# ShuoYangRobotics/Cerberus

Measured on NVIDIA H100. Metric: sliding-window solves/sec (10-frame x 150-feature windows), higher is better.
Workload: dtype f64

## Files before the change

### cerberus_b200/csrc/solve_kernel.cuh

```cuda
#pragma once
#include "eval_kernels.cuh"

namespace cerb {

#if defined(CERB_PHASE_TIMING) && !defined(CERB_CUSIM)
__device__ unsigned long long g_phase_cycles[48];
#define PH_DECL() long long ph_t = clock64()
#define PH_MARK_T(id, t) do { if ((threadIdx.x & 31) == 0) { const long long ph_n = clock64(); if (threadIdx.x == (t)) atomicAdd(&g_phase_cycles[id], (unsigned long long)(ph_n - ph_t)); ph_t = ph_n; } __syncwarp(); } while (0)
#define PH_MARK(id) PH_MARK_T(id, 0)
#define PH_ARG , long long &ph_t
#define PH_FWD , ph_t
#else
#define PH_DECL()
#define PH_MARK_T(id, t)
#define PH_MARK(id)
#define PH_ARG
#define PH_FWD
#endif

enum { CERB_WINDOW = 10, NX = 79, NYB = 13, NFR = 11, NY = 143, NR = 222, NRP = 224, HXX_SZ = 79 * 79, HXY_SZ = 79 * 143, X_TD = 78, SOLVE_THREADS = 256, FT = 64, TILE_LD = 33, NOBS_PLANES = 9 };
enum { HBLK = NYB * NYB, AD_SZ = NFR * HBLK, BO_SZ = (NFR - 1) * HBLK };
#ifndef CERB_SOLVE_MIN_BLOCKS
#define CERB_SOLVE_MIN_BLOCKS 1
#endif
// ... 53 lines not shown
    double *red;
    double *wj;
    double *sca;
    double *chain_col;
    double *idg;
    double *idx;
    int *ti;
    unsigned long long *mbar;
    double *tile;
};
enum { S_RADIUS = 0, S_MU, S_REUSE, S_XCOST, S_CCOST, S_ALPHA, S_GNORM2, S_GNNORM2, S_GDOTGN, S_MODEL, S_STEPNORM, S_XNORM, S_DLNORM,
       S_OK, S_DONE, S_TERM, S_ITER, S_NSUCC, S_INVALID, S_GMAX, S_INIT_COST, S_P, S_Q, S_VHV, S_LCOST, S_LNORM, S_LGMAX, S_COUNT };
static_assert(S_COUNT <= 32, "scalar slots overlap the chain's column line");
enum { TI_PRIOR_MAP = 0, TI_NCHUNKS = 96, TI_CHUNK_CACHE = 97, TI_CACHED_CHUNKS = 15, TI_CHAIN_DONE = 130, TI_IMU_MASK = 131, TI_INTS = 132 };
static_assert(TI_PRIOR_MAP + CERB_MAX_PRIOR_DIM <= TI_NCHUNKS && TI_CHUNK_CACHE + 2 * TI_CACHED_CHUNKS <= TI_CHAIN_DONE && TI_IMU_MASK < TI_INTS && TI_INTS % 2 == 0,
              "s.ti slots overlap");
enum { SMEM_DOUBLES = HXX_SZ + SMEM_HXX_PAD + HXY_SZ + AD_SZ + BO_SZ + 7 * NRP + 2 * ST_STRIDE + 99 + 18 + 3 + 31 * 39 + 960 + 192 + 8 * 256 + 128 * 8 + 32 + 32 + TI_INTS / 2 + 144 + 80 };

CERB_D void smem_carve(double *base, Smem &s) {
    double *p = base;
    s.Hxx = p; p += HXX_SZ; s.mbar = reinterpret_cast<unsigned long long *>(p + 1); p += SMEM_HXX_PAD; s.Hxy = p; p += HXY_SZ; s.Ad = p; p += AD_SZ; s.Bo = p; p += BO_SZ;
    s.g = p; p += NRP; s.sc = p; p += NRP; s.D = p; p += NRP; s.gh = p; p += NRP; s.gn = p; p += NRP; s.stp = p; p += NRP; s.yv = p; p += NRP;
    s.xs = p; p += ST_STRIDE; s.xc = p; p += ST_STRIDE;
    s.Rw = p; p += 99; s.Rex = p; p += 18; p += 3;
    s.Ju = p; p += 31 * 39; s.red = p; p += 8 * 256; s.wj = p; p += 128 * 8;
    s.lin = p; p += 960; s.pdx = p; p += 96; s.pr = p; p += 96; s.sca = p; p += 32; s.chain_col = p; p += 32;
    s.ti = reinterpret_cast<int *>(p); p += TI_INTS / 2;
    s.idg = p; p += 144;
    s.idx = p; p += 80;
    s.tile = s.Hxy;
}

template <int NV>
CERB_D void block_sum(const double *v, double *red, double *out, int tid) {
    for (int k = 0; k < NV; k++) red[k * 256 + tid] = v[k];
    __syncthreads();
    for (int s = 128; s > 0; s >>= 1) {
        if (tid < s) for (int k = 0; k < NV; k++) red[k * 256 + tid] += red[k * 256 + tid + s];
        __syncthreads();
    }
    for (int k = 0; k < NV; k++) out[k] = red[k * 256];
    __syncthreads();
}

CERB_D void copy_g2s(double *dst, const double *src, int n, int tid) {
    for (int k0 = tid; k0 < n; k0 += 8 * SOLVE_THREADS) {
        double b[8];
        _Pragma("unroll")
        for (int u = 0; u < 8; u++) { const int k = k0 + u * SOLVE_THREADS; b[u] = (k < n) ? src[k] : 0.0; }
        _Pragma("unroll")
        for (int u = 0; u < 8; u++) { const int k = k0 + u * SOLVE_THREADS; if (k < n) dst[k] = b[u]; }
    }
}
CERB_D void copy_g2s_async(double *dst, const double *src, int n, int tid) {
    for (int k = tid; k < n; k += SOLVE_THREADS) CERB_CP_ASYNC8(dst + k, src + k);
}
CERB_D void load_geometry(const double *x, Smem &s, int tid) {
    if (tid < 11) { const m33 R = qtoR(ldq(x + ST_POSE + 7 * tid + 3)); for (int k = 0; k < 9; k++) s.Rw[9 * tid + k] = R.m[k]; }
    else if (tid < 13) { const int e = tid - 11; const m33 R = qtoR(ldq(x + ST_EX + 7 * e + 3)); for (int k = 0; k < 9; k++) s.Rex[9 * e + k] = R.m[k]; }
    __syncthreads();
}

struct ObsCtx { int start, nobs, off; double lam, pix, piy, vix, viy, tdi; };

struct ObsVals { double px, py, vx, vy, td; int stereo; };
CERB_D void obs_fetch(const double *obs, const int *stereo, int mo, int o, int cam, ObsVals &v) {
    v.px = obs[(cam ? 4 : 0) * mo + o]; v.py = obs[(cam ? 5 : 1) * mo + o]; v.vx = obs[(cam ? 6 : 2) * mo + o]; v.vy = obs[(cam ? 7 : 3) * mo + o];
    v.td = obs[8 * mo + o]; v.stereo = stereo[o];
}

CERB_NOINLINE double vision_cost(const SolveParams &P, int w, const double *x, const double *lam, int tid) {
    CERB_DYN_SMEM(double, smem_base);
    Smem s; smem_carve(smem_base, s);
    const int nF = P.n_features[w], mo = P.maxObs;
    const double *obs = P.obs + (size_t)w * NOBS_PLANES * P.maxObs;
    const int *stereo = P.obs_stereo + (size_t)w * P.maxObs;
    double cost = 0.0;
    for (int idx = tid; idx < 4 * nF; idx += SOLVE_THREADS) {
        const int f = idx >> 2, cam = idx & 1, part = (idx >> 1) & 1;
        ObsCtx c;
        c.start = P.feat_start[(size_t)w * P.maxF + f]; c.nobs = P.feat_nobs[(size_t)w * P.maxF + f]; c.off = P.feat_off[(size_t)w * P.maxF + f];
        c.lam = lam[f];
        c.pix = obs[0 * mo + c.off]; c.piy = obs[1 * mo + c.off]; c.vix = obs[2 * mo + c.off]; c.viy = obs[3 * mo + c.off];
        c.tdi = obs[8 * mo + c.off];
        const int k0 = part ? 6 : 0, k1 = part ? c.nobs : (c.nobs < 6 ? c.nobs : 6);
        const double inv_l = 1.0 / c.lam;
        const int i = c.start;
        const d3 tic = ld3(x + ST_EX);
        const double tdv = x[ST_TD];
        const d3 pts_i_td = mk3(c.pix, c.piy, 1.0) - (tdv - c.tdi) * mk3(c.vix, c.viy, 0.0);
        const d3 p_bi = mv33(ldm33(s.Rex), inv_l * pts_i_td) + tic;
        const d3 p_w = mv33(ldm33(s.Rw + 9 * i), p_bi) + ld3(x + ST_POSE + 7 * i);
        const double *Rcp = cam ? s.Rex + 9 : s.Rex;
        const d3 tc = cam ? ld3(x + ST_EX + 7) : tic;
        ObsVals cur, nxt;
        cur.px = cur.py = cur.vx = cur.vy = cur.td = 0.0; cur.stereo = 0;
        if (k0 < k1) obs_fetch(obs, stereo, mo, c.off + k0, cam, cur);
        _Pragma("unroll 1")
        for (int k = k0; k < k1; k++) {
            nxt = cur;
            if (k + 1 < k1) obs_fetch(obs, stereo, mo, c.off + k + 1, cam, nxt);
            const bool k3 = (k == 0);
            const bool on = k3 ? (cam == 1 && cur.stereo) : (cam == 0 || cur.stereo);
            if (on) {
                const int j = c.start + k;
                const d3 p_bj = k3 ? p_bi : mTv33(ldm33(s.Rw + 9 * j), p_w - ld3(x + ST_POSE + 7 * j));
                const d3 p_cj = mTv33(ldm33(Rcp), p_bj - tc);
                const double iz = 1.0 / p_cj.z;
                const double r0 = P.sqrt_info * (p_cj.x * iz - (cur.px - (tdv - cur.td) * cur.vx));
// ... 243 lines not shown
            PH_MARK(29);
            __syncthreads();
            PH_MARK(22);
            if (jbase >= 0) {
                _Pragma("unroll")
                for (int fj = 0; fj < 2; fj++) {
                    const int jf = j0 + fj;
                    if (jf >= NFR || jf == a) continue;
                    const double *q = jp + (4 * fj) * VJ_SZ + tid;
                    smem_base[jbase + jca * a + jcj * jf] += ((q[0] + q[VJ_SZ]) + q[2 * VJ_SZ]) + q[3 * VJ_SZ];
                }
            }
            PH_MARK(23);
        }
        __syncthreads();
        {
            double *ex = T;
            ex[0 * 256 + tid] = h; ex[1 * 256 + tid] = gq; ex[2 * 256 + tid] = wT;
            for (int k = 0; k < 6; k++) { ex[(3 + k) * 256 + tid] = wI[k]; ex[(9 + k) * 256 + tid] = wE0[k]; ex[(15 + k) * 256 + tid] = wE1[k]; }
        }
        __syncthreads();
        for (int e = tid; e < VP_SZ; e += SOLVE_THREADS) {
            double v = 0.0;
            for (int wq = 0; wq < 8; wq++) v += ((wq < 5) ? s.Ju + 8 * VJ_SZ + VP_SZ * wq : s.tile + VT_SZ + VP_SZ * (wq - 5))[e];
            const int blk = e >> 6, ra = (e >> 3) & 7, rb = e & 7;
            const int ga = blk < 3 ? 0 : (blk < 5 ? 2 : 3), gb = blk == 0 ? 0 : (blk == 1 || blk == 3 ? 2 : 3);
            vis_scatter(s, ga, gb, ra, rb, a, a, v);
        }
        if (tid < 64 && ev) {
            const double *ex = T;
            double q[21];
            for (int k = 0; k < 21; k++) q[k] = ((ex[k * 256 + tid] + ex[k * 256 + 64 + tid]) + ex[k * 256 + 128 + tid]) + ex[k * 256 + 192 + tid];
            hh[f] = q[0] * slf * slf; gl[f] = q[1] * slf;
            W[(size_t)X_TD * F + f] = q[2] * (prescale ? s.sc[X_TD] * slf : 1.0);
            for (int k = 0; k < 6; k++) {
                W[(size_t)(6 * a + k) * F + f] = q[3 + k] * (prescale ? s.sc[6 * a + k] * slf : 1.0);
                W[(size_t)(66 + k) * F + f] = q[9 + k] * (prescale ? s.sc[66 + k] * slf : 1.0);
                W[(size_t)(72 + k) * F + f] = q[15 + k] * (prescale ? s.sc[72 + k] * slf : 1.0);
            }
        }
        __syncthreads();
        PH_MARK(24);
    }
    return cost;
}

CERB_D void imu_lin_all(const SolveParams &P, Smem &s, int w, const double *x, bool want_jac, int tid) {
    if (tid < CERB_WINDOW) {
        const double *pre = P.pre + ((size_t)w * CERB_WINDOW + tid) * PRE_STRIDE;
        IMULegLin *L = reinterpret_cast<IMULegLin *>(s.lin + 96 * tid);
        imu_leg_linearize(pre, x + ST_POSE + 7 * tid, x + ST_SB + 9 * tid, x + ST_LB + 4 * tid, x + ST_POSE + 7 * (tid + 1),
                          x + ST_SB + 9 * (tid + 1), x + ST_LB + 4 * (tid + 1), P.G, want_jac, L);
    }
    __syncthreads();
}

CERB_D double prior_residual(const SolveParams &P, Smem &s, int w, const double *x, int tid) {
    const int *meta = P.prior_meta + (size_t)w * PRIOR_META_STRIDE;
    if (!meta[0]) return 0.0;
    const int n = meta[1], nb = meta[2];
    const double *J = P.prior_J + (size_t)w * PRIOR_LD * PRIOR_LD, *r0 = P.prior_r + (size_t)w * PRIOR_LD, *x0 = P.prior_x0 + (size_t)w * 16 * 9;
    if (tid < nb) {
        const int kind = meta[4 + 3 * tid], index = meta[5 + 3 * tid], col = meta[6 + 3 * tid];
        prior_block_dx(kind, x + prior_block_state_offset(kind, index), x0 + 9 * tid, s.pdx + col);
    }
    __syncthreads();
    int parts = SOLVE_THREADS / n; if (parts > 4) parts = 4; if (parts < 1) parts = 1;
    const int kc = (n + parts - 1) / parts;
    double *part = s.red;
    for (int e = tid; e < parts * n; e += SOLVE_THREADS) {
        const int p = e / n, i = e % n;
        const int k1 = (p + 1) * kc < n ? (p + 1) * kc : n;
        double t = 0.0;
        for (int k = p * kc; k < k1; k++) t += J[(size_t)k * n + i] * s.pdx[k];
        part[p * PRIOR_LD + i] = t;
    }
    __syncthreads();
    double cost = 0.0;
    for (int i = tid; i < n; i += SOLVE_THREADS) {
        double t = r0[i];
        for (int p = 0; p < parts; p++) t += part[p * PRIOR_LD + i];
        s.pr[i] = t; cost += 0.5 * t * t;
    }
    __syncthreads();
    return cost;
}

CERB_NOINLINE double inertial_cost(const SolveParams &P, int w, const double *x, int tid) {
    CERB_DYN_SMEM(double, smem_base);
    Smem s; smem_carve(smem_base, s);
    imu_lin_all(P, s, w, x, false, tid);
    double cost = 0.0;
    for (int idx = tid; idx < CERB_WINDOW * 31; idx += SOLVE_THREADS) {
        const int i = idx / 31, r = idx % 31;
        const double *pre = P.pre + ((size_t)w * CERB_WINDOW + i) * PRE_STRIDE;
        if (pre[PRE_SUM_DT] > 10.0) continue;
        const double *ru = s.lin + 96 * i, *S = P.sinfo + ((size_t)w * CERB_WINDOW + i) * 961;
        double t = 0.0;
        for (int q = r; q < 31; q++) t += S[r * 31 + q] * ru[q];
        cost += 0.5 * t * t;
    }
    return cost + prior_residual(P, s, w, x, tid);
}

CERB_D int imu_col_dest(int i, int c) {
    if (c < 6) return 6 * i + c;
    if (c < 19) return -(1 + NYB * i + (c - 6));
    if (c < 25) return 6 * (i + 1) + (c - 19);
    return -(1 + NYB * (i + 1) + (c - 25));
}
CERB_D void scatter_addr(const Smem &s, int da, int db, double **a0, double **a1) {
    *a1 = nullptr;
    if (da >= 0 && db >= 0) { *a0 = (da <= db) ? s.Hxx + da * NX + db : s.Hxx + db * NX + da; return; }
    if (da >= 0) { *a0 = s.Hxy + da * NY + (-db - 1); return; }
    if (db >= 0) { *a0 = s.Hxy + db * NY + (-da - 1); return; }
    const int ya = -da - 1, yb = -db - 1;
    const int fa = ya / NYB, fb = yb / NYB, ka = ya % NYB, kb = yb % NYB;
    if (fa == fb) { *a0 = s.Ad + fa * HBLK + ka * NYB + kb; if (ka != kb) *a1 = s.Ad + fa * HBLK + kb * NYB + ka; }
    else if (fb == fa + 1) *a0 = s.Bo + fa * HBLK + ka * NYB + kb;
    else *a0 = s.Bo + fb * HBLK + kb * NYB + ka;
}
CERB_D void scatter_H(Smem &s, int da, int db, double v) {
    if (da >= 0 && db >= 0) { if (da <= db) s.Hxx[da * NX + db] += v; else s.Hxx[db * NX + da] += v; return; }
    if (da >= 0) { s.Hxy[da * NY + (-db - 1)] += v; return; }
    if (db >= 0) { s.Hxy[db * NY + (-da - 1)] += v; return; }
    const int ya = -da - 1, yb = -db - 1;
    const int fa = ya / NYB, fb = yb / NYB, ka = ya % NYB, kb = yb % NYB;
    if (fa == fb) { s.Ad[fa * HBLK + ka * NYB + kb] += v; if (ka != kb) s.Ad[fa * HBLK + kb * NYB + ka] += v; }
    else if (fb == fa + 1) s.Bo[fa * HBLK + ka * NYB + kb] += v;
    else s.Bo[fb * HBLK + kb * NYB + ka] += v;
}

enum { IMU_LDJ = 44, IMU_TILE = 32 * 44, IMU_WARPS = 3, PRIOR_THREADS = SOLVE_THREADS - 32 * IMU_WARPS };
CERB_NOINLINE double inertial_linearize(const SolveParams &P, int w, const double *x, int tid) {
    CERB_DYN_SMEM(double, smem_base);
    Smem s; smem_carve(smem_base, s);
    double cost = 0.0;
    PH_DECL();
    imu_lin_all(P, s, w, x, true, tid);
    PH_MARK(25);
    const int wid = tid >> 5, lane = tid & 31;
    CERB_CP_ASYNC_WAIT();
    double *gp = s.stp;
    double *ppart = s.yv;
    for (int k = tid; k < NRP; k += SOLVE_THREADS) gp[k] = 0.0;
    __syncthreads();
    if (wid < IMU_WARPS) {
        double *Jt = s.Ju + IMU_TILE * wid;
        int plx[30], ply[30];
        {
            const int *plan = ws_carve(P).imu_plan;
            _Pragma("unroll")
            for (int q = 0; q < 30; q++) { plx[q] = __ldg(plan + (2 * q) * 32 + lane); ply[q] = __ldg(plan + (2 * q + 1) * 32 + lane); }
            const int dummy = (int)(s.idg - smem_base) + lane;
            _Pragma("unroll")
            for (int q = 0; q < 30; q++) if (plx[q] == dummy && (ply[q] & 4095) == 0) plx[q] += 32 * wid;
        }
        double sa[20];
        auto load_S = [&](int i) {
            const double *S = P.sinfo + ((size_t)w * CERB_WINDOW + i) * 961;
            int q = 0;
            _Pragma("unroll")
            for (int mi = 0; mi < 4; mi++)
                _Pragma("unroll")
                for (int ks = 2 * mi; ks < 8; ks++) {
                    const int r = 8 * mi + (lane >> 2), c = 4 * ks + (lane & 3);
                    sa[q++] = (r < 31 && c < 31 && c >= r) ? S[r * 31 + c] : 0.0;
                }
        };
        load_S(wid * 4);
        const int imu_mask = s.ti[TI_IMU_MASK];
        double sdt[4];
        _Pragma("unroll")
        for (int rnd = 0; rnd < 4; rnd++) { const int i = rnd + 4 * wid; sdt[rnd] = (i < CERB_WINDOW) ? P.pre[((size_t)w * CERB_WINDOW + i) * PRE_STRIDE + PRE_SUM_DT] : 1e30; }
        _Pragma("unroll")
        for (int rnd = 0; rnd < 4; rnd++) {
            const int i = rnd + 4 * wid;
            const double *pre = P.pre + ((size_t)w * CERB_WINDOW + (i < CERB_WINDOW ? i : 0)) * PRE_STRIDE;
            if (i < CERB_WINDOW && !(sdt[rnd] > 10.0) && (imu_mask == 0 || (imu_mask == 1 && i == 0))) {
                for (int k = lane; k < IMU_TILE; k += 32) Jt[k] = 0.0;
                __syncwarp();
                if (lane < 11) imu_leg_fill_ju_part(*reinterpret_cast<const IMULegLin *>(s.lin + 96 * i), pre, Jt, IMU_LDJ, lane);
                if (lane < 31) Jt[lane * IMU_LDJ + 38] = s.lin[96 * i + lane];
                __syncwarp();
                PH_MARK(32);
                for (int ni = 0; ni < 5; ni++) {
                    double b[8];
                    _Pragma("unroll")
                    for (int ks = 0; ks < 8; ks++) b[ks] = Jt[(4 * ks + (lane & 3)) * IMU_LDJ + 8 * ni + (lane >> 2)];
                    __syncwarp();
                    double c[4][2];
                    int q = 0;
                    _Pragma("unroll")
                    for (int mi = 0; mi < 4; mi++) {
                        c[mi][0] = 0.0; c[mi][1] = 0.0;
                        _Pragma("unroll")
                        for (int ks = 2 * mi; ks < 8; ks++) { CERB_DMMA(c[mi][0], c[mi][1], sa[q], b[ks], c[mi][0], c[mi][1]); q++; }
                    }
                    _Pragma("unroll")
                    for (int mi = 0; mi < 4; mi++) { double *o = Jt + (8 * mi + (lane >> 2)) * IMU_LDJ + 8 * ni + 2 * (lane & 3); o[0] = c[mi][0]; o[1] = c[mi][1]; }
                    __syncwarp();
                }
                PH_MARK(33);
                if (i + 1 < CERB_WINDOW && rnd < 3) load_S(i + 1);
                double acc[15][2];
                _Pragma("unroll")
                for (int k = 0; k < 15; k++) { acc[k][0] = 0.0; acc[k][1] = 0.0; }
                for (int ks = 0; ks < 8; ks++) {
                    double f[5];
                    _Pragma("unroll")
                    for (int n = 0; n < 5; n++) f[n] = Jt[(4 * ks + (lane & 3)) * IMU_LDJ + 8 * n + (lane >> 2)];
                    int q = 0;
                    _Pragma("unroll")
                    for (int mi = 0; mi < 5; mi++)
                        _Pragma("unroll")
                        for (int ni = mi; ni < 5; ni++) { CERB_DMMA(acc[q][0], acc[q][1], f[mi], f[ni], acc[q][0], acc[q][1]); q++; }
                }
                PH_MARK(34);
                if (lane == 27) cost += 0.5 * acc[14][0];
                _Pragma("unroll")
                for (int hq = 0; hq < 30; hq += 15) {
                    double cur[15];
                    _Pragma("unroll")
                    for (int t = 0; t < 15; t++) cur[t] = smem_base[plx[hq + t] + i * (ply[hq + t] & 4095)];
                    _Pragma("unroll")
                    for (int t = 0; t < 15; t++) {
                        const int o = plx[hq + t] + i * (ply[hq + t] & 4095);
                        const double nv = cur[t] + acc[(hq + t) >> 1][(hq + t) & 1];
                        smem_base[o] = nv;
                        smem_base[o + (ply[hq + t] >> 12) - 256] = nv;
                    }
                }
                PH_MARK(35);
            } else if (i + 1 < CERB_WINDOW && rnd < 3) load_S(i + 1);
            CERB_BAR_SYNC(2, 32 * IMU_WARPS);
            PH_MARK(36);
        }
        PH_MARK(30);
    } else {
        const int *meta = P.prior_meta + (size_t)w * PRIOR_META_STRIDE;
        if (meta[0]) {
            const int t5 = tid - 32 * IMU_WARPS, n = meta[1], nb = meta[2];
            const double *J = P.prior_J + (size_t)w * PRIOR_LD * PRIOR_LD, *r0 = P.prior_r + (size_t)w * PRIOR_LD, *x0 = P.prior_x0 + (size_t)w * 16 * 9;
            if (t5 < nb) {
                const int kind = meta[4 + 3 * t5], index = meta[5 + 3 * t5], col = meta[6 + 3 * t5];
                prior_block_dx(kind, x + prior_block_state_offset(kind, index), x0 + 9 * t5, s.pdx + col);
            }
            CERB_BAR_SYNC(3, PRIOR_THREADS);
            const int kc = (n + 1) / 2;
            for (int e = t5; e < 2 * n; e += PRIOR_THREADS) {
                const int p = e / n, i = e % n;
                const int k1 = (p + 1) * kc < n ? (p + 1) * kc : n;
                double t = 0.0;
                for (int k = p * kc; k < k1; k++) t += J[(size_t)k * n + i] * s.pdx[k];
                ppart[p * PRIOR_LD + i] = t;
            }
            CERB_BAR_SYNC(3, PRIOR_THREADS);
            for (int i = t5; i < n; i += PRIOR_THREADS) {
                const double t = (r0[i] + ppart[i]) + ppart[PRIOR_LD + i];
                s.pr[i] = t; cost += 0.5 * t * t;
            }
            CERB_BAR_SYNC(3, PRIOR_THREADS);
            for (int c = wid - IMU_WARPS; c < n; c += PRIOR_THREADS / 32) {
                double t = 0.0;
                for (int k = lane; k < n; k += 32) t += J[(size_t)c * n + k] * s.pr[k];
                for (int o = 16; o > 0; o >>= 1) t += __shfl_sync(0xffffffffu, t, (lane + o) & 31);
                const int d = s.ti[TI_PRIOR_MAP + c];
                if (lane == 0) gp[d >= 0 ? d : NX + (-d - 1)] += t;
            }
        }
        PH_MARK_T(31, 96);
    }
    __syncthreads();
    PH_MARK(26);
    for (int k = tid; k < NR; k += SOLVE_THREADS) s.g[k] += gp[k];
    __syncthreads();
    PH_MARK(27);
    return cost;
}

CERB_D void apply_plus(const Smem &s, const double *delta, const double *lam, const double *dlam, double *lamc, int nF, bool ex_open, bool td_open, int tid) {
    if (tid < 11) pose_plus(s.xs + ST_POSE + 7 * tid, delta + 6 * tid, s.xc + ST_POSE + 7 * tid);
    else if (tid < 13) {
        const int e = tid - 11;
        if (ex_open) pose_plus(s.xs + ST_EX + 7 * e, delta + 66 + 6 * e, s.xc + ST_EX + 7 * e);
        else for (int k = 0; k < 7; k++) s.xc[ST_EX + 7 * e + k] = s.xs[ST_EX + 7 * e + k];
    }
    for (int k = tid; k < 99; k += SOLVE_THREADS) { const int f = k / 9, c = k % 9; s.xc[ST_SB + k] = s.xs[ST_SB + k] + delta[NX + NYB * f + c]; }
    for (int k = tid; k < 44; k += SOLVE_THREADS) { const int f = k / 4, c = k % 4; s.xc[ST_LB + k] = s.xs[ST_LB + k] + delta[NX + NYB * f + 9 + c]; }
    if (tid == 0) s.xc[ST_TD] = td_open ? s.xs[ST_TD] + delta[X_TD] : s.xs[ST_TD];
    for (int f = tid; f < nF; f += SOLVE_THREADS) lamc[f] = lam[f] + dlam[f];
    __syncthreads();
}

CERB_D double ambient_sq(const double *a, const double *b, const double *la, const double *lb, int nF, bool ex_open, bool lb_open, bool td_open, int tid) {
    double t = 0.0;
    for (int k = tid; k < ST_SIZE; k += SOLVE_THREADS) {
        if (k >= ST_LB && k < ST_EX && !lb_open) continue;
        if (k >= ST_EX && k < ST_TD && !ex_open) continue;
        if (k == ST_TD && !td_open) continue;
        const double v = b ? a[k] - b[k] : a[k];
        t += v * v;
    }
    for (int f = tid; f < nF; f += SOLVE_THREADS) { const double v = lb ? la[f] - lb[f] : la[f]; t += v * v; }
    return t;
}

template <bool SUB>
CERB_D double w_column_dot(const double *wf, int F, const double *v, double t) {
    constexpr int BATCH = 16;
    for (int a0 = 0; a0 < NX; a0 += BATCH) {
        double wr[BATCH];
        _Pragma("unroll")
        for (int u = 0; u < BATCH; u++) wr[u] = (a0 + u < NX) ? wf[(size_t)(a0 + u) * F] : 0.0;
        _Pragma("unroll")
        for (int u = 0; u < BATCH; u++) {
            if (a0 + u < NX) { if (SUB) t -= wr[u] * v[a0 + u]; else t += wr[u] * v[a0 + u]; }
        }
    }
    return t;
}

template <int W> struct TTPlan;
#define CERB_TT_PLAN(W, NR_, NB_, ...) template <> struct TTPlan<W> { static constexpr int nr = NR_, nb = NB_; static CERB_HD int tab(int i) { constexpr int t[] = {__VA_ARGS__}; return t[i]; } };
CERB_TT_PLAN(0, 4, 7, 0, 1, 2, 3, 0, 0, 0,   0, 0, 1, 0, 1, 0, 1,   0, 1, 1, 2, 2, 3, 3)
CERB_TT_PLAN(1, 4, 7, 2, 3, 4, 5, 0, 0, 0,   0, 0, 1, 0, 1, 0, 1,   0, 1, 1, 2, 2, 3, 3)
CERB_TT_PLAN(2, 4, 7, 4, 5, 6, 7, 0, 0, 0,   0, 0, 1, 0, 1, 0, 1,   0, 1, 1, 2, 2, 3, 3)
// ... 114 lines not shown
    }
    return has_prior;
}

CERB_D void build_imu_plan(const Smem &s, const double *smem_base, int *plan, int tid) {
    if (tid >= 32) return;
    int q = 0;
    for (int mi = 0; mi < 5; mi++)
        for (int ni = mi; ni < 5; ni++, q++)
            for (int e = 0; e < 2; e++) {
                const int la = 8 * mi + (tid >> 2), lb = 8 * ni + 2 * (tid & 3) + e;
                int px = (int)(s.idg - smem_base) + tid, py = 256 << 12;
                if (la <= lb && lb <= 38 && la != 38) {
                    double *p0[2], *p1[2];
                    for (int i = 0; i < 2; i++) {
                        const int da = imu_col_dest(i, la);
                        if (lb == 38) { p0[i] = da >= 0 ? s.g + da : s.g + NX + (-da - 1); p1[i] = nullptr; }
                        else scatter_addr(s, da, imu_col_dest(i, lb), &p0[i], &p1[i]);
                    }
                    px = (int)(p0[0] - smem_base);
                    py = (int)(p0[1] - p0[0]) | (((p1[0] ? (int)(p1[0] - p0[0]) : 0) + 256) << 12);
                }
                plan[(2 * (q * 2 + e)) * 32 + tid] = px; plan[(2 * (q * 2 + e) + 1) * 32 + tid] = py;
            }
}
CERB_D void build_chunks(const int *fstart, Smem &s, int *chunks, int n_end) {
    int n = 0, c0 = 0;
    while (c0 < n_end) {
        chunks[1 + n] = c0;
        const int a = fstart[c0];
        int e = c0 + 1;
        while (e < n_end && e < c0 + 64 && fstart[e] == a) e++;
        if (n < TI_CACHED_CHUNKS) { s.ti[TI_CHUNK_CACHE + 2 * n] = c0; s.ti[TI_CHUNK_CACHE + 2 * n + 1] = ((e - c0) << 8) | a; }
        n++; c0 = e;
    }
    chunks[1 + n] = n_end; chunks[0] = n; s.ti[TI_NCHUNKS] = n;
}
struct Win { int w, nF; bool ex_open, lb_open, td_open, has_prior, bulk_ok; double *lam; CtaWs ws; };
struct PriorCopy { unsigned par0, par1; bool hxx_prefetched; };
CERB_D void linearize(const SolveParams &P, Smem &s, const Win &c, PriorCopy &pc, const double *xl, const double *laml, bool first, int tid PH_ARG) {
    const int F = c.ws.F, nF = c.nF;
    double *sca = s.sca, *W = c.ws.W, *hh = c.ws.hh, *gl = c.ws.gl, *sl = c.ws.sl, *pimg = c.ws.pimg;
    if (!c.has_prior) { for (int k = tid; k < HXX_SZ; k += SOLVE_THREADS) s.Hxx[k] = 0.0; }
    else if (c.bulk_ok) {
        if (!pc.hxx_prefetched) { __syncthreads(); if (tid == 0) CERB_BULK_G2S(s.Hxx, pimg, PIMG_HXY * 8, &s.mbar[0]); }
        CERB_MBAR_WAIT(&s.mbar[0], pc.par0); pc.par0 ^= 1;
    } else { if (!pc.hxx_prefetched) copy_g2s_async(s.Hxx, pimg, HXX_SZ, tid); CERB_CP_ASYNC_WAIT(); }
    pc.hxx_prefetched = false;
    for (int k = tid; k < NRP; k += SOLVE_THREADS) s.g[k] = 0.0;
    load_geometry(xl, s, tid);
    double part[2];
    PH_MARK(0);
    part[0] = vision_linearize(P, c.w, xl, laml, W, hh, gl, sl, !first, c.ws.chunks, tid);
    if (c.has_prior && c.bulk_ok) {
        if (tid == 0) CERB_BULK_G2S(s.Hxy, pimg + PIMG_HXY, PIMG_REST * 8, &s.mbar[1]);
        CERB_MBAR_WAIT(&s.mbar[1], pc.par1); pc.par1 ^= 1;
    } else if (c.has_prior) copy_g2s_async(s.Hxy, pimg + PIMG_HXY, PIMG_REST, tid);
    else for (int k = tid; k < PIMG_REST; k += SOLVE_THREADS) s.Hxy[k] = 0.0;
    __syncthreads();
    PH_MARK(1);
    part[0] += inertial_linearize(P, c.w, xl, tid);
    PH_MARK(2);
    part[1] = ambient_sq(xl, nullptr, laml, nullptr, nF, c.ex_open, c.lb_open, c.td_open, tid);
    double tot[2];
    block_sum<2>(part, s.red, tot, tid);
    if (tid == 0) { sca[S_LCOST] = tot[0]; sca[S_LNORM] = sqrt(tot[1]); }
    if (first) {
        for (int k = tid; k < NR; k += SOLVE_THREADS) {
            double d;
            bool active = true;
            if (k < NX) { d = s.Hxx[k * NX + k]; if (k >= 66 && k < X_TD && !c.ex_open) active = false; if (k == X_TD && !c.td_open) active = false; }
            else { const int yk = k - NX, f = yk / NYB, q = yk % NYB; d = s.Ad[f * HBLK + q * NYB + q]; if (q >= 9 && !c.lb_open) active = false; }
            s.sc[k] = active ? 1.0 / (1.0 + sqrt(d)) : 0.0;
        }
        for (int f = tid; f < nF; f += SOLVE_THREADS) sl[f] = 1.0 / (1.0 + sqrt(hh[f]));
    }
    __syncthreads();
    if (P.dbg && c.w == P.dbg_window && first) {
        for (int k = tid; k < NR; k += SOLVE_THREADS) {
            int dst; double d;
            if (k < NX) { dst = k < X_TD ? k : 221; d = s.Hxx[k * NX + k]; }
            else { const int yk = k - NX, f = yk / NYB, q = yk % NYB; dst = q < 9 ? 78 + 9 * f + q : 177 + 4 * f + (q - 9); d = s.Ad[f * HBLK + q * NYB + q]; }
            const bool act = s.sc[k] != 0.0;
            P.dbg[1 + dst] = act ? s.g[k] : 0.0; P.dbg[1 + NR + F + dst] = act ? d : 0.0;
        }
        for (int f = tid; f < nF; f += SOLVE_THREADS) { P.dbg[1 + NR + f] = gl[f]; P.dbg[1 + NR + F + NR + f] = hh[f]; }
        if (tid == 0) P.dbg[0] = sca[S_LCOST];
    }
    double gm = 0.0;
    for (int k = tid; k < NR; k += SOLVE_THREADS) if (s.sc[k] != 0.0) gm = fmax(gm, fabs(s.g[k]));
    for (int f = tid; f < nF; f += SOLVE_THREADS) gm = fmax(gm, fabs(!first ? gl[f] / sl[f] : gl[f]));
    for (int o = 16; o > 0; o >>= 1) gm = fmax(gm, __shfl_sync(0xffffffffu, gm, (tid + o) & 31));
    if ((tid & 31) == 0) s.red[tid >> 5] = gm;
    __syncthreads();
    if (tid == 0) { double m8 = s.red[0]; for (int k = 1; k < SOLVE_THREADS / 32; k++) m8 = fmax(m8, s.red[k]); sca[S_LGMAX] = m8; }
    for (int a = tid >> 5; a < NX; a += SOLVE_THREADS / 32) {
        const double sa = s.sc[a];
        for (int b = a + (tid & 31); b < NX; b += 32) { const double v = s.Hxx[a * NX + b] * (sa * s.sc[b]); s.Hxx[a * NX + b] = v; s.Hxx[b * NX + a] = v; }
        for (int q = tid & 31; q < NY; q += 32) s.Hxy[a * NY + q] *= sa * s.sc[NX + q];
    }
    for (int k = tid; k < AD_SZ; k += SOLVE_THREADS) { const int f = k / HBLK, a = (k % HBLK) / NYB, b = k % NYB; s.Ad[k] *= s.sc[NX + NYB * f + a] * s.sc[NX + NYB * f + b]; }
    for (int k = tid; k < BO_SZ; k += SOLVE_THREADS) { const int f = k / HBLK, a = (k % HBLK) / NYB, b = k % NYB; s.Bo[k] *= s.sc[NX + NYB * f + a] * s.sc[NX + NYB * (f + 1) + b]; }
    for (int k = tid; k < NR; k += SOLVE_THREADS) s.g[k] *= s.sc[k];
    if (first) {
        for (int k = tid; k < NX * nF; k += SOLVE_THREADS) { const int a = k / nF, f = k % nF; W[(size_t)a * F + f] *= s.sc[a] * sl[f]; }
        for (int f = tid; f < nF; f += SOLVE_THREADS) { hh[f] *= sl[f] * sl[f]; gl[f] *= sl[f]; }
    }
    __syncthreads();
}
CERB_D bool finalize_iteration(const SolveParams &P, double *sca, int iteration, int tid) {
    if (tid == 0) {
        if (iteration >= P.max_iters) { sca[S_DONE] = 1; sca[S_TERM] = 1; }
        else if (sca[S_GMAX] <= P.gtol) { sca[S_DONE] = 1; sca[S_TERM] = 0; }
        else if (sca[S_RADIUS] <= P.min_radius) { sca[S_DONE] = 1; sca[S_TERM] = 0; }
// ... 568 lines not shown
}

struct MargParams {
    const int *flags;
    const double *state, *lam;
    double *A, *b;
    int posmax;
    int *dims;
    int *blocks;
};
enum { MARG_OLD = 0, MARG_SECOND_NEW = 1 };

CERB_GLOBAL void __launch_bounds__(SOLVE_THREADS, 1) marg_assemble_kernel(CERB_GRID_CONSTANT SolveParams P, CERB_GRID_CONSTANT MargParams M) {
    CERB_DYN_SMEM(double, smem_base);
    Smem s; smem_carve(smem_base, s);
    const int tid = threadIdx.x, F = P.maxF;
    const CtaWs ws = ws_carve(P);
    int *colx = reinterpret_cast<int *>(s.idx);
    int *coly = colx + 80;
    int *misc = coly + 32;
    build_imu_plan(s, smem_base, ws.imu_plan, tid);
    __syncthreads();
    for (int w = blockIdx.x; w < P.n_windows; w += gridDim.x) {
        const int nF = P.n_features[w], flag = M.flags[w];
        const double *lam = M.lam + (size_t)w * F;
        const int *pmeta = P.prior_meta + (size_t)w * PRIOR_META_STRIDE;
        const int *fstart = P.feat_start + (size_t)w * F, *fnobs = P.feat_nobs + (size_t)w * F, *foff = P.feat_off + (size_t)w * F;
        const int *stereo = P.obs_stereo + (size_t)w * P.maxObs;
        if (tid == 0) {
            int n0 = 0;
            if (flag == MARG_OLD) while (n0 < nF && fstart[n0] == 0) n0++;
            build_chunks(fstart, s, ws.chunks, n0);
            s.ti[TI_IMU_MASK] = flag == MARG_OLD ? 1 : 2;
            misc[0] = n0; misc[4] = 0; misc[5] = 0;
        }
        const bool has_prior = build_prior_image(P, s, w, ws.pimg, tid);
        for (int k = tid; k < ST_STRIDE; k += SOLVE_THREADS) s.xs[k] = (k < ST_SIZE) ? M.state[(size_t)w * ST_STRIDE + k] : 0.0;
        __syncthreads();
        const int n0 = misc[0];
        {
            int st = 0, len = 0;
            for (int f = tid; f < n0; f += SOLVE_THREADS) { const int nb = fnobs[f]; len = nb > len ? nb : len; for (int k = 0; k < nb; k++) st |= (stereo[foff[f] + k] != 0); }
            s.red[tid] = (double)(len | (st << 8));
            __syncthreads();
            if (tid == 0) { int l = 0, q = 0; for (int k = 0; k < SOLVE_THREADS; k++) { const int v = (int)s.red[k]; l = (v & 255) > l ? (v & 255) : l; q |= v >> 8; } misc[4] = q; misc[5] = l; }
            __syncthreads();
        }
        if (!has_prior) { for (int k = tid; k < HXX_SZ; k += SOLVE_THREADS) s.Hxx[k] = 0.0; }
        else copy_g2s(s.Hxx, ws.pimg, HXX_SZ, tid);
        for (int k = tid; k < NRP; k += SOLVE_THREADS) s.g[k] = 0.0;
        load_geometry(s.xs, s, tid);
        if (n0 > 0) vision_linearize(P, w, s.xs, lam, ws.W, ws.hh, ws.gl, ws.sl, false, ws.chunks, tid);
        __syncthreads();
        if (has_prior) copy_g2s(s.Hxy, ws.pimg + PIMG_HXY, PIMG_REST, tid);
        else for (int k = tid; k < PIMG_REST; k += SOLVE_THREADS) s.Hxy[k] = 0.0;
        __syncthreads();
        inertial_linearize(P, w, s.xs, tid);
        if (tid == 0) {
            bool pose[NFR] = {false}, sb[2] = {false, false}, lb[2] = {false, false}, ex[2] = {false, false}, td = false;
            if (has_prior) for (int b = 0; b < pmeta[2]; b++) {
                const int kind = pmeta[4 + 3 * b], index = pmeta[5 + 3 * b];
                if (kind == 0) pose[index] = true; else if (kind == 1) sb[index ? 1 : 0] = true; else if (kind == 2) lb[index ? 1 : 0] = true;
                else if (kind == 3) ex[index] = true; else td = true;
            }
            const bool noleg = (P.flags[w] & 4) != 0;
            if (flag == MARG_OLD) {
                if (!(P.pre[(size_t)w * CERB_WINDOW * PRE_STRIDE + PRE_SUM_DT] > 10.0)) { pose[0] = pose[1] = true; sb[0] = sb[1] = true; if (!noleg) lb[0] = lb[1] = true; }
                if (n0 > 0) { pose[0] = true; ex[0] = true; td = true; if (misc[4]) ex[1] = true; for (int j = 1; j < misc[5] && j < NFR; j++) pose[j] = true; }
            }
            for (int k = 0; k < 80 + 32; k++) colx[k] = -1;
            int m = 0, n = 0, status = 1, nblk = 0;
            int *blk = M.blocks + (size_t)w * 64;
#define MARG_BLK(kind_, shifted_, src_) do { blk[4 * nblk] = (kind_); blk[4 * nblk + 1] = (shifted_); blk[4 * nblk + 2] = n; blk[4 * nblk + 3] = (src_); nblk++; } while (0)
            if (flag == MARG_OLD) {
                if (pose[0]) { for (int k = 0; k < 6; k++) colx[k] = m + k; m += 6; }
                if (sb[0]) { for (int k = 0; k < 9; k++) coly[k] = m + k; m += 9; }
                if (lb[0]) { for (int k = 0; k < 4; k++) coly[9 + k] = m + k; m += 4; }
                m += n0;
                if (m == 0) status = 0;
                for (int j = 1; j < NFR; j++) if (pose[j]) { for (int k = 0; k < 6; k++) colx[6 * j + k] = m + n + k; MARG_BLK(0, j - 1, j); n += 6; }
                if (sb[1]) { for (int k = 0; k < 9; k++) coly[13 + k] = m + n + k; MARG_BLK(1, 0, 1); n += 9; }
                if (lb[1]) { for (int k = 0; k < 4; k++) coly[13 + 9 + k] = m + n + k; MARG_BLK(2, 0, 1); n += 4; }
            } else {
                if (!has_prior || !pose[CERB_WINDOW - 1]) status = 2;
                else {
                    for (int k = 0; k < 6; k++) colx[6 * (CERB_WINDOW - 1) + k] = k;
                    m = 6;
                    for (int j = 0; j < NFR; j++) if (pose[j] && j != CERB_WINDOW - 1) {
                        for (int k = 0; k < 6; k++) colx[6 * j + k] = m + n + k;
                        MARG_BLK(0, (j == CERB_WINDOW) ? j - 1 : j, j); n += 6;
                    }
                    if (sb[0]) { for (int k = 0; k < 9; k++) coly[k] = m + n + k; MARG_BLK(1, 0, 0); n += 9; }
                    if (lb[0]) { for (int k = 0; k < 4; k++) coly[9 + k] = m + n + k; MARG_BLK(2, 0, 0); n += 4; }
                }
            }
            if (status == 1) {
                for (int e = 0; e < 2; e++) if (ex[e]) { for (int k = 0; k < 6; k++) colx[66 + 6 * e + k] = m + n + k; MARG_BLK(3, e, e); n += 6; }
                if (td) { colx[X_TD] = m + n; MARG_BLK(4, 0, 0); n += 1; }
            }
#undef MARG_BLK
            misc[1] = m; misc[2] = n; misc[3] = status;
            int *dm = M.dims + 4 * w; dm[0] = m; dm[1] = n; dm[2] = status; dm[3] = nblk;
        }
        __syncthreads();
        if (misc[3] == 1) {
            const int m = misc[1], n = misc[2], pos = m + n, l0 = m - n0;
            double *A = M.A + (size_t)w * M.posmax * M.posmax, *b = M.b + (size_t)w * M.posmax;
            for (int e = tid; e < pos * pos; e += SOLVE_THREADS) A[e] = 0.0;
            __syncthreads();
            for (int e = tid; e < NX * NX; e += SOLVE_THREADS) {
// ... 30 lines not shown
```

Measured before the change: 34830.

## Restructure inertial linearization to spread IMU squaring across all warps before loading prior image

The inertial linearization now runs the per-frame IMU Jacobian squaring across all eight warps instead of three. It uses the Hxy region as scratch before the prior image is loaded, and parks the results of the first two frames in shared memory. The load of the prior Hxy/Hyy image, bulk or async, is deferred until after the tensor-core work, so that tile space can be reused and the copy overlaps less critical work. The prior Jacobian is also staged into shared memory with cp.async for both prior matvecs. This adds a parked-fragment buffer and more complex multi-round scatter synchronization, at the cost of extra __syncthreads per scatter round.

```diff
diff --git a/cerberus_b200/csrc/solve_kernel.cuh b/cerberus_b200/csrc/solve_kernel.cuh
--- a/cerberus_b200/csrc/solve_kernel.cuh
+++ b/cerberus_b200/csrc/solve_kernel.cuh
@@ -129,9 +129,10 @@
         for (int u = 0; u < 8; u++) { const int k = k0 + u * SOLVE_THREADS; if (k < n) dst[k] = b[u]; }
     }
 }
-CERB_D void copy_g2s_async(double *dst, const double *src, int n, int tid) {
-    for (int k = tid; k < n; k += SOLVE_THREADS) CERB_CP_ASYNC8(dst + k, src + k);
-}
+CERB_D void copy_g2s_async_part(double *dst, const double *src, int n, int t, int nthreads) {
+    for (int k = t; k < n; k += nthreads) CERB_CP_ASYNC8(dst + k, src + k);
+}
+CERB_D void copy_g2s_async(double *dst, const double *src, int n, int tid) { copy_g2s_async_part(dst, src, n, tid, SOLVE_THREADS); }
 CERB_D void load_geometry(const double *x, Smem &s, int tid) {
     if (tid < 11) { const m33 R = qtoR(ldq(x + ST_POSE + 7 * tid + 3)); for (int k = 0; k < 9; k++) s.Rw[9 * tid + k] = R.m[k]; }
     else if (tid < 13) { const int e = tid - 11; const m33 R = qtoR(ldq(x + ST_EX + 7 * e + 3)); for (int k = 0; k < 9; k++) s.Rex[9 * e + k] = R.m[k]; }
@@ -481,7 +482,6 @@
         imu_leg_linearize(pre, x + ST_POSE + 7 * tid, x + ST_SB + 9 * tid, x + ST_LB + 4 * tid, x + ST_POSE + 7 * (tid + 1),
                           x + ST_SB + 9 * (tid + 1), x + ST_LB + 4 * (tid + 1), P.G, want_jac, L);
     }
-    __syncthreads();
 }
 
 CERB_D double prior_residual(const SolveParams &P, Smem &s, int w, const double *x, int tid) {
@@ -519,6 +519,7 @@
     CERB_DYN_SMEM(double, smem_base);
     Smem s; smem_carve(smem_base, s);
     imu_lin_all(P, s, w, x, false, tid);
+    __syncthreads();
     double cost = 0.0;
     for (int idx = tid; idx < CERB_WINDOW * 31; idx += SOLVE_THREADS) {
         const int i = idx / 31, r = idx % 31;
@@ -560,128 +561,48 @@
     else s.Bo[fb * HBLK + kb * NYB + ka] += v;
 }
 
-enum { IMU_LDJ = 44, IMU_TILE = 32 * 44, IMU_WARPS = 3, PRIOR_THREADS = SOLVE_THREADS - 32 * IMU_WARPS };
-CERB_NOINLINE double inertial_linearize(const SolveParams &P, int w, const double *x, int tid) {
+enum { IMU_LDJ = 44, IMU_TILE = 32 * 44, IMU_FRAG = 30 * 32, PRIOR_THREADS = SOLVE_THREADS - 96 };
+static_assert(8 * IMU_TILE <= PIMG_REST && 2 * IMU_TILE + PRIOR_LD * PRIOR_LD <= PIMG_REST && 2 * IMU_FRAG + CERB_WINDOW <= 31 * 39 + 8 * 256 + 128 * 8, "IMU tiles / staged J0 / parked fragments");
+CERB_NOINLINE double inertial_linearize(const SolveParams &P, int w, const double *x, const double *prior_rest, int prior_parity, int tid) {
     CERB_DYN_SMEM(double, smem_base);
     Smem s; smem_carve(smem_base, s);
     double cost = 0.0;
     PH_DECL();
-    imu_lin_all(P, s, w, x, true, tid);
-    PH_MARK(25);
     const int wid = tid >> 5, lane = tid & 31;
-    CERB_CP_ASYNC_WAIT();
     double *gp = s.stp;
     double *ppart = s.yv;
-    for (int k = tid; k < NRP; k += SOLVE_THREADS) gp[k] = 0.0;
-    __syncthreads();
-    if (wid < IMU_WARPS) {
-        double *Jt = s.Ju + IMU_TILE * wid;
-        int plx[30], ply[30];
-        {
-            const int *plan = ws_carve(P).imu_plan;
-            _Pragma("unroll")
-            for (int q = 0; q < 30; q++) { plx[q] = __ldg(plan + (2 * q) * 32 + lane); ply[q] = __ldg(plan + (2 * q + 1) * 32 + lane); }
-            const int dummy = (int)(s.idg - smem_base) + lane;
-            _Pragma("unroll")
-            for (int q = 0; q < 30; q++) if (plx[q] == dummy && (ply[q] & 4095) == 0) plx[q] += 32 * wid;
-        }
-        double sa[20];
-        auto load_S = [&](int i) {
-            const double *S = P.sinfo + ((size_t)w * CERB_WINDOW + i) * 961;
-            int q = 0;
-            _Pragma("unroll")
-            for (int mi = 0; mi < 4; mi++)
-                _Pragma("unroll")
-                for (int ks = 2 * mi; ks < 8; ks++) {
-                    const int r = 8 * mi + (lane >> 2), c = 4 * ks + (lane & 3);
-                    sa[q++] = (r < 31 && c < 31 && c >= r) ? S[r * 31 + c] : 0.0;
-                }
-        };
-        load_S(wid * 4);
-        const int imu_mask = s.ti[TI_IMU_MASK];
-        double sdt[4];
-        _Pragma("unroll")
-        for (int rnd = 0; rnd < 4; rnd++) { const int i = rnd + 4 * wid; sdt[rnd] = (i < CERB_WINDOW) ? P.pre[((size_t)w * CERB_WINDOW + i) * PRE_STRIDE + PRE_SUM_DT] : 1e30; }
-        _Pragma("unroll")
-        for (int rnd = 0; rnd < 4; rnd++) {
-            const int i = rnd + 4 * wid;
-            const double *pre = P.pre + ((size_t)w * CERB_WINDOW + (i < CERB_WINDOW ? i : 0)) * PRE_STRIDE;
-            if (i < CERB_WINDOW && !(sdt[rnd] > 10.0) && (imu_mask == 0 || (imu_mask == 1 && i == 0))) {
-                for (int k = lane; k < IMU_TILE; k += 32) Jt[k] = 0.0;
-                __syncwarp();
-                if (lane < 11) imu_leg_fill_ju_part(*reinterpret_cast<const IMULegLin *>(s.lin + 96 * i), pre, Jt, IMU_LDJ, lane);
-                if (lane < 31) Jt[lane * IMU_LDJ + 38] = s.lin[96 * i + lane];
-                __syncwarp();
-                PH_MARK(32);
-                for (int ni = 0; ni < 5; ni++) {
-                    double b[8];
-                    _Pragma("unroll")
-                    for (int ks = 0; ks < 8; ks++) b[ks] = Jt[(4 * ks + (lane & 3)) * IMU_LDJ + 8 * ni + (lane >> 2)];
-                    __syncwarp();
-                    double c[4][2];
-                    int q = 0;
-                    _Pragma("unroll")
-                    for (int mi = 0; mi < 4; mi++) {
-                        c[mi][0] = 0.0; c[mi][1] = 0.0;
-                        _Pragma("unroll")
-                        for (int ks = 2 * mi; ks < 8; ks++) { CERB_DMMA(c[mi][0], c[mi][1], sa[q], b[ks], c[mi][0], c[mi][1]); q++; }
-                    }
-                    _Pragma("unroll")
-                    for (int mi = 0; mi < 4; mi++) { double *o = Jt + (8 * mi + (lane >> 2)) * IMU_LDJ + 8 * ni + 2 * (lane & 3); o[0] = c[mi][0]; o[1] = c[mi][1]; }
-                    __syncwarp();
-                }
-                PH_MARK(33);
-                if (i + 1 < CERB_WINDOW && rnd < 3) load_S(i + 1);
-                double acc[15][2];
-                _Pragma("unroll")
-                for (int k = 0; k < 15; k++) { acc[k][0] = 0.0; acc[k][1] = 0.0; }
-                for (int ks = 0; ks < 8; ks++) {
-                    double f[5];
-                    _Pragma("unroll")
-                    for (int n = 0; n < 5; n++) f[n] = Jt[(4 * ks + (lane & 3)) * IMU_LDJ + 8 * n + (lane >> 2)];
-                    int q = 0;
-                    _Pragma("unroll")
-                    for (int mi = 0; mi < 5; mi++)
-                        _Pragma("unroll")
-                        for (int ni = mi; ni < 5; ni++) { CERB_DMMA(acc[q][0], acc[q][1], f[mi], f[ni], acc[q][0], acc[q][1]); q++; }
-                }
-                PH_MARK(34);
-                if (lane == 27) cost += 0.5 * acc[14][0];
-                _Pragma("unroll")
-                for (int hq = 0; hq < 30; hq += 15) {
-                    double cur[15];
-                    _Pragma("unroll")
-                    for (int t = 0; t < 15; t++) cur[t] = smem_base[plx[hq + t] + i * (ply[hq + t] & 4095)];
-                    _Pragma("unroll")
-                    for (int t = 0; t < 15; t++) {
-                        const int o = plx[hq + t] + i * (ply[hq + t] & 4095);
-                        const double nv = cur[t] + acc[(hq + t) >> 1][(hq + t) & 1];
-                        smem_base[o] = nv;
-                        smem_base[o + (ply[hq + t] >> 12) - 256] = nv;
-                    }
-                }
-                PH_MARK(35);
-            } else if (i + 1 < CERB_WINDOW && rnd < 3) load_S(i + 1);
-            CERB_BAR_SYNC(2, 32 * IMU_WARPS);
-            PH_MARK(36);
-        }
-        PH_MARK(30);
-    } else {
-        const int *meta = P.prior_meta + (size_t)w * PRIOR_META_STRIDE;
+    double *park = s.Ju;
+    double *fcost = s.Ju + 2 * IMU_FRAG;
+    const int *meta = P.prior_meta + (size_t)w * PRIOR_META_STRIDE;
+    const double *J = P.prior_J + (size_t)w * PRIOR_LD * PRIOR_LD;
+    double *sJ = s.Hxy + 2 * IMU_TILE;
+    const int imu_mask = s.ti[TI_IMU_MASK];
+    auto active = [&](int i) {
+        return !(P.pre[((size_t)w * CERB_WINDOW + i) * PRE_STRIDE + PRE_SUM_DT] > 10.0) && (imu_mask == 0 || (imu_mask == 1 && i == 0));
+    };
+    const int i_reg = wid < 2 ? wid + 8 : wid;
+    const int i_park = (wid == 2 || wid == 3) ? wid - 2 : -1;
+    const bool act_first = active(wid), act_reg = active(i_reg), act_park = i_park >= 0 && active(i_park);
+    imu_lin_all(P, s, w, x, true, tid);
+    if (wid >= 3) {
+        const int t5 = tid - 96;
+        for (int k = t5; k < NRP; k += PRIOR_THREADS) gp[k] = 0.0;
         if (meta[0]) {
-            const int t5 = tid - 32 * IMU_WARPS, n = meta[1], nb = meta[2];
-            const double *J = P.prior_J + (size_t)w * PRIOR_LD * PRIOR_LD, *r0 = P.prior_r + (size_t)w * PRIOR_LD, *x0 = P.prior_x0 + (size_t)w * 16 * 9;
+            const int n = meta[1], nb = meta[2];
+            const double *r0 = P.prior_r + (size_t)w * PRIOR_LD, *x0 = P.prior_x0 + (size_t)w * 16 * 9;
+            copy_g2s_async_part(sJ, J, n * n, t5, PRIOR_THREADS);
             if (t5 < nb) {
                 const int kind = meta[4 + 3 * t5], index = meta[5 + 3 * t5], col = meta[6 + 3 * t5];
                 prior_block_dx(kind, x + prior_block_state_offset(kind, index), x0 + 9 * t5, s.pdx + col);
             }
+            CERB_CP_ASYNC_WAIT();
             CERB_BAR_SYNC(3, PRIOR_THREADS);
             const int kc = (n + 1) / 2;
             for (int e = t5; e < 2 * n; e += PRIOR_THREADS) {
                 const int p = e / n, i = e % n;
                 const int k1 = (p + 1) * kc < n ? (p + 1) * kc : n;
                 double t = 0.0;
-                for (int k = p * kc; k < k1; k++) t += J[(size_t)k * n + i] * s.pdx[k];
+                for (int k = p * kc; k < k1; k++) t += sJ[k * n + i] * s.pdx[k];
                 ppart[p * PRIOR_LD + i] = t;
             }
             CERB_BAR_SYNC(3, PRIOR_THREADS);
@@ -689,19 +610,136 @@
                 const double t = (r0[i] + ppart[i]) + ppart[PRIOR_LD + i];
                 s.pr[i] = t; cost += 0.5 * t * t;
             }
-            CERB_BAR_SYNC(3, PRIOR_THREADS);
-            for (int c = wid - IMU_WARPS; c < n; c += PRIOR_THREADS / 32) {
-                double t = 0.0;
-                for (int k = lane; k < n; k += 32) t += J[(size_t)c * n + k] * s.pr[k];
-                for (int o = 16; o > 0; o >>= 1) t += __shfl_sync(0xffffffffu, t, (lane + o) & 31);
-                const int d = s.ti[TI_PRIOR_MAP + c];
-                if (lane == 0) gp[d >= 0 ? d : NX + (-d - 1)] += t;
-            }
-        }
+            PH_MARK_T(41, 96);
+        }
+    }
+    double sa[20];
+    auto load_S = [&](int i) {
+        const double *S = P.sinfo + ((size_t)w * CERB_WINDOW + i) * 961;
+        int q = 0;
+        _Pragma("unroll")
+        for (int mi = 0; mi < 4; mi++)
+            _Pragma("unroll")
+            for (int ks = 2 * mi; ks < 8; ks++) {
+                const int r = 8 * mi + (lane >> 2), c = 4 * ks + (lane & 3);
+                sa[q++] = (r < 31 && c < 31 && c >= r) ? S[r * 31 + c] : 0.0;
+            }
+    };
+    load_S(act_first ? wid : i_reg);
+    __syncthreads();
+    PH_MARK(25);
+    double *Jt = s.Hxy + IMU_TILE * wid;
+    auto square = [&](int i, bool prefetch_next, double (&acc)[15][2]) {
+        const double *pre = P.pre + ((size_t)w * CERB_WINDOW + i) * PRE_STRIDE;
+        for (int k = lane; k < IMU_TILE; k += 32) Jt[k] = 0.0;
+        __syncwarp();
+        if (lane < 11) imu_leg_fill_ju_part(*reinterpret_cast<const IMULegLin *>(s.lin + 96 * i), pre, Jt, IMU_LDJ, lane);
+        if (lane < 31) Jt[lane * IMU_LDJ + 38] = s.lin[96 * i + lane];
+        __syncwarp();
+        PH_MARK(32);
+        for (int ni = 0; ni < 5; ni++) {
+            double b[8];
+            _Pragma("unroll")
+            for (int ks = 0; ks < 8; ks++) b[ks] = Jt[(4 * ks + (lane & 3)) * IMU_LDJ + 8 * ni + (lane >> 2)];
+            __syncwarp();
+            double c[4][2];
+            int q = 0;
+            _Pragma("unroll")
+            for (int mi = 0; mi < 4; mi++) {
+                c[mi][0] = 0.0; c[mi][1] = 0.0;
+                _Pragma("unroll")
+                for (int ks = 2 * mi; ks < 8; ks++) { CERB_DMMA(c[mi][0], c[mi][1], sa[q], b[ks], c[mi][0], c[mi][1]); q++; }
+            }
+            _Pragma("unroll")
+            for (int mi = 0; mi < 4; mi++) { double *o = Jt + (8 * mi + (lane >> 2)) * IMU_LDJ + 8 * ni + 2 * (lane & 3); o[0] = c[mi][0]; o[1] = c[mi][1]; }
+            __syncwarp();
+        }
+        PH_MARK(33);
+        if (prefetch_next) load_S(i_reg);
+        _Pragma("unroll")
+        for (int k = 0; k < 15; k++) { acc[k][0] = 0.0; acc[k][1] = 0.0; }
+        for (int ks = 0; ks < 8; ks++) {
+            double fr[5];
+            _Pragma("unroll")
+            for (int n = 0; n < 5; n++) fr[n] = Jt[(4 * ks + (lane & 3)) * IMU_LDJ + 8 * n + (lane >> 2)];
+            int q = 0;
+            _Pragma("unroll")
+            for (int mi = 0; mi < 5; mi++)
+                _Pragma("unroll")
+                for (int ni = mi; ni < 5; ni++) { CERB_DMMA(acc[q][0], acc[q][1], fr[mi], fr[ni], acc[q][0], acc[q][1]); q++; }
+        }
+        __syncwarp();
+        PH_MARK(34);
+        if (lane == 27) fcost[i] = 0.5 * acc[14][0];
+    };
+    if (wid < 2) {
+        if (act_first) {
+            double first[15][2];
+            square(wid, act_reg, first);
+            _Pragma("unroll")
+            for (int q = 0; q < 30; q++) park[(30 * wid + q) * 32 + lane] = first[q >> 1][q & 1];
+        } else if (lane == 27) fcost[wid] = 0.0;
+    }
+    if (wid >= 2 && meta[0]) {
+        const int n = meta[1];
+        for (int c = wid - 2; c < n; c += 6) {
+            double t = 0.0;
+            for (int k = lane; k < n; k += 32) t += sJ[c * n + k] * s.pr[k];
+            for (int o = 16; o > 0; o >>= 1) t += __shfl_sync(0xffffffffu, t, (lane + o) & 31);
+            const int d = s.ti[TI_PRIOR_MAP + c];
+            if (lane == 0) gp[d >= 0 ? d : NX + (-d - 1)] += t;
+        }
+        CERB_BAR_SYNC(2, SOLVE_THREADS - 64);
         PH_MARK_T(31, 96);
     }
-    __syncthreads();
-    PH_MARK(26);
+    double acc[15][2];
+    if (act_reg) square(i_reg, false, acc);
+    else if (lane == 27) fcost[i_reg] = 0.0;
+    __syncthreads();
+    PH_MARK(30);
+    if (lane == 27 && wid < 3) {
+        _Pragma("unroll")
+        for (int r = 0; r < 4; r++) if (4 * wid + r < CERB_WINDOW) cost += fcost[4 * wid + r];
+    }
+    if (!prior_rest) for (int k = tid; k < PIMG_REST; k += SOLVE_THREADS) s.Hxy[k] = 0.0;
+    else if (prior_parity >= 0) { if (tid == 0) CERB_BULK_G2S(s.Hxy, prior_rest, PIMG_REST * 8, &s.mbar[1]); }
+    else copy_g2s_async(s.Hxy, prior_rest, PIMG_REST, tid);
+    if (prior_rest && prior_parity >= 0) CERB_MBAR_WAIT(&s.mbar[1], prior_parity);
+    else CERB_CP_ASYNC_WAIT();
+    __syncthreads();
+    PH_MARK(40);
+    const int *plan = ws_carve(P).imu_plan;
+    const int dummy = (int)(s.idg - smem_base) + lane;
+    _Pragma("unroll 1")
+    for (int rnd = 0; rnd < 4; rnd++) {
+        const bool own = act_reg && (i_reg & 3) == rnd, parked = act_park && i_park == rnd;
+        if (own || parked) {
+            const int i = own ? i_reg : i_park;
+            const double *pk = park + 30 * 32 * (parked ? i_park : 0) + lane;
+            _Pragma("unroll")
+            for (int hq = 0; hq < 30; hq += 15) {
+                int o[15], m[15];
+                double cur[15], add[15];
+                _Pragma("unroll")
+                for (int t = 0; t < 15; t++) {
+                    const int px = __ldg(plan + (2 * (hq + t)) * 32 + lane), py = __ldg(plan + (2 * (hq + t) + 1) * 32 + lane);
+                    o[t] = (px == dummy && (py & 4095) == 0) ? px + 32 * (wid >> 1) : px + i * (py & 4095);
+                    m[t] = (py >> 12) - 256;
+                }
+                _Pragma("unroll")
+                for (int t = 0; t < 15; t++) { cur[t] = smem_base[o[t]]; add[t] = parked ? pk[(hq + t) * 32] : acc[(hq + t) >> 1][(hq + t) & 1]; }
+                _Pragma("unroll")
+                for (int t = 0; t < 15; t++) {
+                    const double nv = cur[t] + add[t];
+                    smem_base[o[t]] = nv;
+                    smem_base[o[t] + m[t]] = nv;
+                }
+            }
+        }
+        PH_MARK(35);
+        __syncthreads();
+        PH_MARK(36);
+    }
     for (int k = tid; k < NR; k += SOLVE_THREADS) s.g[k] += gp[k];
     __syncthreads();
     PH_MARK(27);
@@ -922,14 +960,10 @@
     double part[2];
     PH_MARK(0);
     part[0] = vision_linearize(P, c.w, xl, laml, W, hh, gl, sl, !first, c.ws.chunks, tid);
-    if (c.has_prior && c.bulk_ok) {
-        if (tid == 0) CERB_BULK_G2S(s.Hxy, pimg + PIMG_HXY, PIMG_REST * 8, &s.mbar[1]);
-        CERB_MBAR_WAIT(&s.mbar[1], pc.par1); pc.par1 ^= 1;
-    } else if (c.has_prior) copy_g2s_async(s.Hxy, pimg + PIMG_HXY, PIMG_REST, tid);
-    else for (int k = tid; k < PIMG_REST; k += SOLVE_THREADS) s.Hxy[k] = 0.0;
-    __syncthreads();
     PH_MARK(1);
-    part[0] += inertial_linearize(P, c.w, xl, tid);
+    const bool bulk = c.has_prior && c.bulk_ok;
+    part[0] += inertial_linearize(P, c.w, xl, c.has_prior ? pimg + PIMG_HXY : nullptr, bulk ? (int)pc.par1 : -1, tid);
+    if (bulk) pc.par1 ^= 1;
     PH_MARK(2);
     part[1] = ambient_sq(xl, nullptr, laml, nullptr, nF, c.ex_open, c.lb_open, c.td_open, tid);
     double tot[2];
@@ -1604,10 +1638,7 @@
         load_geometry(s.xs, s, tid);
         if (n0 > 0) vision_linearize(P, w, s.xs, lam, ws.W, ws.hh, ws.gl, ws.sl, false, ws.chunks, tid);
         __syncthreads();
-        if (has_prior) copy_g2s(s.Hxy, ws.pimg + PIMG_HXY, PIMG_REST, tid);
-        else for (int k = tid; k < PIMG_REST; k += SOLVE_THREADS) s.Hxy[k] = 0.0;
-        __syncthreads();
-        inertial_linearize(P, w, s.xs, tid);
+        inertial_linearize(P, w, s.xs, has_prior ? ws.pimg + PIMG_HXY : nullptr, -1, tid);
         if (tid == 0) {
             bool pose[NFR] = {false}, sb[2] = {false, false}, lb[2] = {false, false}, ex[2] = {false, false}, td = false;
             if (has_prior) for (int b = 0; b < pmeta[2]; b++) {
```

Measured after the change: 35790 (median of 6 runs). 1.03x the previous value.
